# tprodanov/locityper

Hardware: AMD Instinct MI355X
Metric: reads/s through the whole genotyping path (scored + prefiltered + default solver scheme); reads_scored_per_s and genotypes_solved_per_s give the two halves (higher is better)
Workload: dtype f64

## Files before the change

### locityper_amd/csrc/lcty_api.hip

```cpp
#include <algorithm>
#include <cmath>
#include <memory>
#include <numeric>

#include "lcty_objects.hpp"

using namespace lcty;

namespace lcty {
static thread_local std::string g_last_error;
thread_local hipStream_t tl_stream = nullptr;
void set_last_error(const std::string& msg) { g_last_error = msg; }
}

hipEvent_t lcty_ctx::get_event() {
    hipEvent_t e;
    if (!event_pool.empty()) { e = event_pool.back(); event_pool.pop_back(); return e; }
    LCTY_HIP(hipEventCreate(&e));
    return e;
}

void lcty_ctx::fold_oldest(lcty::KernelTimer& t, size_t count) {
    count = std::min(count, t.pending.size());
    for (size_t i = 0; i < count; i++) {
        float ms = 0.f;
        LCTY_HIP(hipEventSynchronize(t.pending[i].second));
        LCTY_HIP(hipEventElapsedTime(&ms, t.pending[i].first, t.pending[i].second));
        t.total_ms += ms; t.launches++;
        event_pool.push_back(t.pending[i].first); event_pool.push_back(t.pending[i].second);
    }
    t.pending.erase(t.pending.begin(), t.pending.begin() + static_cast<std::ptrdiff_t>(count));
}

extern "C" {

int32_t lcty_ctx_set_knob(lcty_ctx* ctx, const char* name, int64_t value) {
    return guarded([&] {
        if (!ctx || !name) fail(LCTY_ERR_INVALID_INPUT, "null argument");
        static const char* const known[] = {"transfer_levels", "transfer_scratch_mb", "transfer_waves", "transfer_cap_new", "transfer_arena",
                                            "depth_table_start", "solve_budget_mb", "solve_chains_per_wave", "solve_extra_start", "solve_lds_weights",
                                            "anneal_lds_weights", "contig_info_slide", "gather_chunk_mb", "prefilter_gram", "prefilter_gram_cols",
                                            "prefilter_gram_levels", "comm_fail_at", "score_lean", "arena_cap_pct", "exact_threads", "host_threads",
                                            "score_lean_keep", "score_lean_two", "queue_early_head",
#ifdef LCTY_DIAG
                                            "solve_stats", "queue_trace", "map_trace", "exact_trace", "solve_greedy_form", "solve_anneal_timing", "score_timing",
                                            "solve_init_tiles", "transfer_phases",
#endif
                                            nullptr};
        bool ok = false;
        for (const char* const* k = known; *k; k++) ok |= strcmp(*k, name) == 0;
        if (!ok) fail(LCTY_ERR_INVALID_INPUT, "unknown knob '%s'", name);
        if (value < 0) ctx->knobs.erase(name); else ctx->knobs[name] = value;
    });
}

int32_t lcty_ctx_set_path(lcty_ctx* ctx, const char* name, const char* path) {
    return guarded([&] {
        if (!ctx || !name) fail(LCTY_ERR_INVALID_INPUT, "null argument");
        if (strcmp(name, "exact_dump") != 0) fail(LCTY_ERR_INVALID_INPUT, "unknown path '%s'", name);
        ctx->exact_dump_path = path ? path : "";
    });
}

const char* lcty_last_error(void) { return g_last_error.c_str(); }
const char* lcty_version(void) { return "locityper_hip 0.1.0 (gfx950)"; }

int32_t lcty_device_count(void) {
    int n = 0;
    if (hipGetDeviceCount(&n) != hipSuccess) { (void)hipGetLastError(); return 0; }
    return n;
}

int32_t lcty_ctx_create(int32_t device_id, lcty_ctx** out) {
    return guarded([&] {
        if (!out) fail(LCTY_ERR_INVALID_INPUT, "null argument");
        int n = 0;
        if (hipGetDeviceCount(&n) != hipSuccess || n == 0) {
            (void)hipGetLastError();
            fail(LCTY_ERR_RUNTIME, "no HIP device is visible: liblocityper_hip has no CPU fallback");
        }
        if (device_id < 0 || device_id >= n) fail(LCTY_ERR_INVALID_INPUT, "device %d out of range (0..%d)", device_id, n - 1);
        auto c = std::unique_ptr<lcty_ctx>(new lcty_ctx());
        c->device = device_id;
        LCTY_HIP(hipSetDevice(device_id));
        LCTY_HIP(hipGetDeviceProperties(&c->props, device_id));
        LCTY_HIP(hipStreamCreateWithFlags(&c->stream.main, hipStreamNonBlocking));
        *out = c.release();
    });
}

void lcty_ctx_destroy(lcty_ctx* ctx) {
    if (!ctx) return;
    (void)hipSetDevice(ctx->device);
    (void)hipStreamSynchronize(ctx->stream);
    for (auto& t : ctx->timers) for (auto& pr : t.pending) { (void)hipEventDestroy(pr.first); (void)hipEventDestroy(pr.second); }
    for (auto e : ctx->event_pool) (void)hipEventDestroy(e);
    if (ctx->gate.ev) (void)hipEventDestroy(ctx->gate.ev);
    if (ctx->gate.init_ev) (void)hipEventDestroy(ctx->gate.init_ev);
    if (ctx->side) { (void)hipStreamSynchronize(ctx->side); (void)hipStreamDestroy(ctx->side); }
    if (ctx->fore) { (void)hipStreamSynchronize(ctx->fore); (void)hipStreamDestroy(ctx->fore); }
    for (auto& slot : ctx->given_slots) if (slot->stream) { (void)hipStreamSynchronize(slot->stream); (void)hipStreamDestroy(slot->stream); }
    (void)hipStreamDestroy(ctx->stream.main);
    delete ctx;
}

int32_t lcty_ctx_synchronize(lcty_ctx* ctx) {
    return guarded([&] {
        if (!ctx) fail(LCTY_ERR_INVALID_INPUT, "null argument");
        ctx->activate();
        LCTY_HIP(hipStreamSynchronize(ctx->stream));
        if (ctx->side) LCTY_HIP(hipStreamSynchronize(ctx->side));
    });
}

int32_t lcty_host_alloc(lcty_ctx* ctx, uint64_t bytes, void** out) {
    return guarded([&] {
        if (!ctx || !out) fail(LCTY_ERR_INVALID_INPUT, "null argument");
        ctx->activate();
        *out = nullptr;
        LCTY_HIP(hipHostMalloc(out, std::max<uint64_t>(bytes, 1), hipHostMallocDefault));
    });
}

void lcty_host_free(void* p) {
    if (p) (void)hipHostFree(p);
}

int32_t lcty_ctx_trim(lcty_ctx* ctx) {
    return guarded([&] {
// ... 282 lines not shown
```

### locityper_amd/csrc/lcty_solve_kernels.hip

```cpp
#include <algorithm>
#include <cmath>
#include <type_traits>
#include <vector>

#include "lcty_solve_device.hpp"

namespace lcty {


__global__ __launch_bounds__(256) void build_loc_table_kernel(const uint32_t* __restrict__ good_ix, uint32_t n_good, uint64_t ngp,
                                                              uint32_t A, const uint32_t* __restrict__ pa_idx,
                                                              const uint64_t* __restrict__ pa_off, const PairAlnDev* __restrict__ pa,
                                                              const double* __restrict__ unmapped, LocCell* __restrict__ table,
                                                              uint32_t* __restrict__ table_ext, double* __restrict__ table_unm,
                                                              uint32_t* __restrict__ err) {
    __shared__ LocCell tile[32][33];
    __shared__ uint32_t tile_ext[32][33];
    const uint32_t g0 = blockIdx.x * 32, c0 = blockIdx.y * 32;
    const uint32_t tx = threadIdx.x & 31u, ty = threadIdx.x >> 5;
    if (blockIdx.y == 0 && threadIdx.x < 32) {
        const uint32_t g = g0 + threadIdx.x;
        if (g < ngp) table_unm[g] = g < n_good ? unmapped[good_ix[g]] : 0.0;
    }
    for (uint32_t i = ty; i < 32; i += 8) {
// ... 338 lines not shown
    for (uint32_t base = seg_lo; base < seg_hi; base += 64) {
        const uint32_t rp = base + lane;
        LocCell cur[P]; uint64_t at[P];
#pragma unroll
        for (uint32_t p = 0; p < P; p++) { cur[p] = nxt[p]; at[p] = row_at[p] + rp; }
        const double cur_unm = nxt_unm;
        if (rp + 64 < seg_hi) {
#pragma unroll
            for (uint32_t p = 0; p < P; p++) nxt[p] = V.table[row_at[p] + rp + 64];
            nxt_unm = V.table_unm[rp + 64];
        }
        Locs<P> L; L.nw = 0;
        uint32_t a0 = 0;
        if (rp < seg_hi) {
            locs_from_cells<P>(L, V, cur, cur_unm, at);
            if (L.nw > 255) atomicMax(V.overflow, 2u);
            if (L.nw > 1 && random_start)
                a0 = static_cast<uint32_t>(__umul64hi(counter_u64(seed ^ INIT_KEY_XOR, rp), static_cast<uint64_t>(L.nw)));
        }
        const bool nontrivial = L.nw > 1;
        const uint32_t n_extra = L.nw > 2 ? min(L.nw, 255u) - 2u : 0u;
        const unsigned long long nt_mask = __ballot(nontrivial);
        const uint32_t slot = n_recs + static_cast<uint32_t>(__popcll(nt_mask & ((1ull << lane) - 1ull)));
        n_recs += static_cast<uint32_t>(__popcll(nt_mask));
        if (L.nw > 0) {
            uint32_t eix = 0;
            if (n_extra) eix = atomicAdd(&seg_cnt[4], n_extra);
            ChainRec rec; rec.rp_cur = rp | (a0 << 24); rec.meta = min(L.nw, 255u) | (eix << 8);
            rec.lp0 = rec.lp1 = 0.0; rec.win0 = rec.win1 = 0;
            const bool room = static_cast<uint64_t>(eix) + n_extra <= V.extra_cap;
            LocIter<P> it; it.start(L);
            LocOut o;
            for (uint32_t t = 0; t < min(L.nw, 255u) && it.next(L, V, o); t++) {
                uint32_t wa, wb;
                loc_windows(V, G, o, seed, rp, t, &wa, &wb);
                const uint32_t win = wa | (wb << 16);
                if (t == 0) { rec.lp0 = o.lp; rec.win0 = win; }
                else if (t == 1) { rec.lp1 = o.lp; rec.win1 = win; }
                else if (room) { ExtraLoc e; e.lp = o.lp; e.win = win; e._pad = 0; extra[eix + t - 2] = e; }
                if (t == a0) {
                    atomicAdd(&depth[wa], 1u);
                    atomicAdd(&depth[wb], 1u);
                    aln_part += o.lp;
                }
            }
            if (nontrivial) recs[slot] = rec;
        }
    }
    if (lane == 0) seg_cnt[wave] = n_recs;
    red[tid] = aln_part;
    __syncthreads();
    const uint32_t ex_total = seg_cnt[4];
    if (tid == 0) {
        if (ex_total > V.extra_cap) { atomicMax(V.overflow, 4u); atomicMax(V.overflow + 1, ex_total); }
        if (ex_total >= (1u << 24)) atomicMax(V.overflow, 2u);
    }
    for (uint32_t s = 128; s > 0; s >>= 1) {
        if (tid < s) red[tid] += red[tid + s];
        __syncthreads();
    }
    uint32_t* gdepth = V.c_depth + static_cast<uint64_t>(chain) * V.wstride;
    for (uint32_t w = tid; w < G.total_w; w += 256) gdepth[w] = depth[w];
    if (tid == 0) {
        uint32_t* cum = V.c_seg + static_cast<uint64_t>(chain) * 4;
        uint32_t run = 0;
        for (uint32_t k = 0; k < INIT_SEGS; k++) { cum[k] = run; run += seg_cnt[k]; }
        V.c_aln[chain] = red[0]; V.c_nnt[chain] = run; V.c_totw[chain] = G.total_w;
    }
}

__device__ __forceinline__ uint64_t counter_fin(uint64_t z) {
    z = (z ^ (z >> 30)) * 0xbf58476d1ce4e5b9ull;
    z = (z ^ (z >> 27)) * 0x94d049bb133111ebull;
    return z ^ (z >> 31);
}
constexpr uint64_t GOLDEN64 = 0x9e3779b97f4a7c15ull;
typedef uint32_t u32x4_t __attribute__((ext_vector_type(4)));
__device__ __forceinline__ void store_16(uint4* p, uint4 v) {
    u32x4_t x; x.x = v.x; x.y = v.y; x.z = v.z; x.w = v.w;
    __builtin_nontemporal_store(x, reinterpret_cast<u32x4_t*>(p));
}
__host__ __device__ inline size_t init_tile_lds(uint32_t T, uint32_t R, uint32_t wstride) {
    const size_t depth = (static_cast<size_t>(T) * wstride * 4 + 15) & ~static_cast<size_t>(15);
    return depth + static_cast<size_t>(T) * 256 * 8 + 4ull * R * 64 * 16 + static_cast<size_t>(T) * 4 * 8 + static_cast<size_t>(T) * 4 * 5 + 64;
}

__device__ __forceinline__ void init_tile_deferred(const SolveView& V, const InitChainP* __restrict__ cp, uint32_t T, uint32_t* depth, double* aln_def,
                                                   uint32_t* ex_cnt, unsigned long long* queue, uint32_t head, uint32_t n, uint32_t wave, uint32_t lane, bool random_start) {
    double add = 0.0;
    uint32_t my_c = 0xFFFFFFFFu;
    if (lane < n) {
        const unsigned long long packed = __hip_atomic_load(&queue[(head + lane) & (INIT_TILE_Q - 1)], __ATOMIC_RELAXED, __HIP_MEMORY_SCOPE_WORKGROUP);
        const uint2 item = make_uint2(static_cast<uint32_t>(packed), static_cast<uint32_t>(packed >> 32));
        const uint32_t c = item.x >> 24, rp = item.x & 0xFFFFFFu, slot = item.y;
        const InitChainP P = cp[c];
        Geno<2> G;
        G.id[0] = P.id0; G.id[1] = P.id1; G.row[0] = P.row0; G.row[1] = P.row1; G.shift[0] = P.shift0; G.shift[1] = P.shift1;
        G.reg_start[0] = P.rs0; G.reg_start[1] = P.rs1; G.reg_end[0] = P.re0; G.reg_end[1] = P.re1; G.total_w = P.total_w;
        Locs<2> L;
        locs_init<2>(L, V, rp, G);
        if (L.nw > 255) atomicMax(V.overflow, 2u);
        uint32_t a0 = 0;
        if (L.nw > 1 && random_start)
            a0 = static_cast<uint32_t>(__umul64hi(counter_u64(P.seed ^ INIT_KEY_XOR, rp), static_cast<uint64_t>(L.nw)));
        const uint32_t nloc = min(L.nw, 255u), n_extra = nloc > 2 ? nloc - 2u : 0u;
        uint32_t eix = 0;
        if (n_extra) eix = atomicAdd(&ex_cnt[c], n_extra);
        const bool room = static_cast<uint64_t>(eix) + n_extra <= V.extra_cap;
        ExtraLoc* extra = V.extra + static_cast<uint64_t>(P.chain) * V.extra_cap;
        ChainRec rec; rec.rp_cur = rp | (a0 << 24); rec.meta = nloc | (eix << 8);
        rec.lp0 = rec.lp1 = 0.0; rec.win0 = rec.win1 = 0;
        LocIter<2> it; it.start(L);
        LocOut o;
        for (uint32_t t = 0; t < nloc && it.next(L, V, o); t++) {
            uint32_t wa, wb;
            loc_windows(V, G, o, P.seed, rp, t, &wa, &wb);
            const uint32_t win = wa | (wb << 16);
            if (t == 0) { rec.lp0 = o.lp; rec.win0 = win; }
            else if (t == 1) { rec.lp1 = o.lp; rec.win1 = win; }
            else if (room) { ExtraLoc e; e.lp = o.lp; e.win = win; e._pad = 0; extra[eix + t - 2] = e; }
            if (t == a0) {
                atomicAdd(&depth[static_cast<size_t>(c) * V.wstride + wa], 1u);
                atomicAdd(&depth[static_cast<size_t>(c) * V.wstride + wb], 1u);
                add = o.lp;
                my_c = c;
            }
        }
        if (L.nw > 1) V.recs[static_cast<uint64_t>(P.chain) * V.rstride + static_cast<uint64_t>(wave) * V.seg_reads + slot] = rec;
    }
    for (uint32_t c = 0; c < T; c++) {
        unsigned long long m = __ballot(my_c == c);
        if (!m) continue;
        double acc = aln_def[c * 4 + wave];
        while (m) {
            const int l = __ffsll(static_cast<long long>(m)) - 1;
            acc += __hiloint2double(__builtin_amdgcn_readlane(__double2hiint(add), l), __builtin_amdgcn_readlane(__double2loint(add), l));
            m &= m - 1;
        }
        if (lane == 0) aln_def[c * 4 + wave] = acc;
    }
}

__global__ __launch_bounds__(256) void solve_init_tile_kernel(const SolveView V, const InitGroup* __restrict__ groups, const InitChainP* __restrict__ chains,
                                                             unsigned long long* lists, const uint32_t T_max, const uint32_t R_max) {
    extern __shared__ __align__(16) uint8_t smem[];
    const uint32_t tid = threadIdx.x, lane = tid & 63u, wave = __builtin_amdgcn_readfirstlane(tid >> 6);
    const InitGroup& grp = groups[blockIdx.x];
    const uint32_t T = grp.n_chains, R = grp.n_rows;
    const InitChainP* __restrict__ cp = chains + grp.first;
    const uint32_t W = V.wstride;
    uint32_t* depth = reinterpret_cast<uint32_t*>(smem);
    size_t at = (static_cast<size_t>(T_max) * W * 4 + 15) & ~static_cast<size_t>(15);
    double* aln = reinterpret_cast<double*>(smem + at); at += static_cast<size_t>(T_max) * 256 * 8;
    uint4* stage = reinterpret_cast<uint4*>(smem + at) + static_cast<size_t>(wave) * R_max * 64; at += 4ull * R_max * 64 * 16;
    unsigned long long* queue = lists + (static_cast<size_t>(blockIdx.x) * 4 + wave) * INIT_TILE_Q;
    double* aln_def = reinterpret_cast<double*>(smem + at); at += static_cast<size_t>(T_max) * 4 * 8;
    uint32_t* ex_cnt = reinterpret_cast<uint32_t*>(smem + at); at += static_cast<size_t>(T_max) * 4;
    uint32_t* seg_cnt = reinterpret_cast<uint32_t*>(smem + at);

    for (uint32_t c = 0; c < T; c++) {
        const InitChainP P = cp[c];
        double* ww = V.c_ww + static_cast<uint64_t>(P.chain) * W;
        uint8_t* wgc = V.c_gc + static_cast<uint64_t>(P.chain) * W;
        uint32_t* wuc = V.n_wk ? V.c_uc + static_cast<uint64_t>(P.chain) * W : nullptr;
        for (uint32_t w = tid; w < P.total_w; w += 256) {
            depth[c * W + w] = 0;
            double weight = 0.0; uint32_t g = 0, uc = V.n_wk - 1;
            if (w >= 2) {
                const bool second = w >= P.shift1;
                const uint32_t allele = second ? P.id1 : P.id0, sh = second ? P.shift1 : P.shift0, rs = second ? P.rs1 : P.rs0;
                const uint32_t start = rs + (w - sh) * V.window, end = start + V.window;
                const uint32_t left = min(V.tweak, start), right = min(V.tweak, V.allele_len[allele] - end);
                const uint64_t r = counter_u64(P.seed ^ WINDOW_KEY_XOR, w);
                const int64_t off = -static_cast<int64_t>(left) + static_cast<int64_t>(__umul64hi(r, static_cast<uint64_t>(left + right + 1)));
                const uint32_t wstart = static_cast<uint32_t>(static_cast<int64_t>(start) + off);
                const uint32_t i = V.ci_off[allele] + (wstart > V.left_padding ? wstart - V.left_padding : 0u);
                weight = V.win_weight[i];
                g = V.gc[i];
                if (wuc) uc = V.uniq_cnt[i] | (static_cast<uint32_t>(V.compl_cnt[i]) << 16);
                if (weight < V.min_weight || weight < 1e-7) { weight = 0.0; g = 0; uc = V.n_wk - 1; }
            }
            ww[w] = weight; wgc[w] = static_cast<uint8_t>(g);
            if (wuc) wuc[w] = uc;
        }
        aln[c * 256 + tid] = 0.0;
        if (tid < 4) aln_def[c * 4 + tid] = 0.0;
        if (tid == 0) ex_cnt[c] = 0;
    }
    __syncthreads();

    const bool random_start = V.solver.kind == LCTY_SOLVER_ANNEAL || (V.solver.kind == LCTY_SOLVER_GREEDY && !V.solver.best_start);
    const uint32_t seg_lo = min(wave * V.seg_reads, V.n_good), seg_hi = min(seg_lo + V.seg_reads, V.n_good);
    uint64_t row_at[INIT_TILE_R];
#pragma unroll
    for (uint32_t r = 0; r < INIT_TILE_R; r++) row_at[r] = static_cast<uint64_t>(grp.row[r < R ? r : 0]) * V.ngp;
    const uint4* __restrict__ table = reinterpret_cast<const uint4*>(V.table);
    uint4 nxt[INIT_TILE_R]; double nxt_unm = 0.0;
#pragma unroll
    for (uint32_t r = 0; r < INIT_TILE_R; r++) nxt[r] = make_uint4(0, 0, 0, 0);
    if (seg_lo + lane < seg_hi) {
#pragma unroll
        for (uint32_t r = 0; r < INIT_TILE_R; r++) if (r < R) nxt[r] = table[row_at[r] + seg_lo + lane];
        nxt_unm = V.table_unm[seg_lo + lane];
    }
    uint32_t n_recs_all = 0;
    uint32_t qn = 0, qhead = 0;
    for (uint32_t base = seg_lo; base < seg_hi; base += 64) {
        const uint32_t rp = base + lane;
        const bool in = rp < seg_hi;
#pragma unroll
        for (uint32_t r = 0; r < INIT_TILE_R; r++) if (r < R) stage[r * 64 + lane] = nxt[r];
        const double unm = nxt_unm;
        if (rp + 64 < seg_hi) {
#pragma unroll
            for (uint32_t r = 0; r < INIT_TILE_R; r++) if (r < R) nxt[r] = table[row_at[r] + rp + 64];
            nxt_unm = V.table_unm[rp + 64];
        }
        const uint64_t zbase = ((static_cast<uint64_t>(rp) << 16) + 1ull) * GOLDEN64;
        const uint64_t abase = (static_cast<uint64_t>(rp) + 1ull) * GOLDEN64;
        for (uint32_t c = 0; c < T; c++) {
            const InitChainP P = cp[c];
            const uint4 qa = stage[P.ia * 64 + lane], qb = stage[P.ib * 64 + lane];
            const double aln_before = aln[c * 256 + tid];
            const double lpA = __hiloint2double(static_cast<int>(qa.y), static_cast<int>(qa.x));
            const double lpB = __hiloint2double(static_cast<int>(qb.y), static_cast<int>(qb.x));
            const uint32_t rawA = qa.z >> 24, rawB = qb.z >> 24;
            const double thresh = fmax(fmax(lpA, lpB), unm) - V.prob_diff;
            const bool kA = in && rawA != 0 && lpA >= thresh, kB = in && rawB != 0 && lpB >= thresh, kU = in && unm >= thresh;
            const bool multi = (kA && rawA > 1) || (kB && rawB > 1);
            const uint32_t nw = (kA ? 1u : 0u) + (kB ? 1u : 0u) + (kU ? 1u : 0u);
            bool nontrivial = nw > 1;
            if (__any(multi && nw == 1)) {
                if (multi && nw == 1) {
                    const uint32_t ext = V.table_ext[static_cast<uint64_t>(kA ? P.row0 : P.row1) * V.ngp + rp];
                    nontrivial = V.pa[ext].ln_prob >= thresh;
                }
            }
            const unsigned long long nt_mask = __ballot(nontrivial);
            const uint32_t before = __builtin_amdgcn_readlane(n_recs_all, c);
            const uint32_t slot = before + static_cast<uint32_t>(__popcll(nt_mask & ((1ull << lane) - 1ull)));
            {
                const uint32_t after = __builtin_amdgcn_readfirstlane(before + static_cast<uint32_t>(__popcll(nt_mask)));
                uint32_t m0_was;
                asm volatile("s_mov_b32 %1, m0\n\ts_mov_b32 m0, %3\n\tv_writelane_b32 %0, %2, m0\n\ts_mov_b32 m0, %1"
                             : "+v"(n_recs_all), "=&s"(m0_was) : "s"(after), "s"(c));
            }
            const unsigned long long mm = __ballot(multi);
            if (mm) {
                if (multi)
                    __hip_atomic_store(&queue[(qhead + qn + static_cast<uint32_t>(__popcll(mm & ((1ull << lane) - 1ull)))) & (INIT_TILE_Q - 1)],
                                       static_cast<unsigned long long>(rp | (c << 24)) | (static_cast<unsigned long long>(slot) << 32), __ATOMIC_RELAXED,
                                       __HIP_MEMORY_SCOPE_WAVEFRONT);
                qn += static_cast<uint32_t>(__popcll(mm));
            }
            const bool BgtA = lpB > lpA, UgtA = unm > lpA, UgtB = unm > lpB;
            const uint32_t posA = ((kB && BgtA) ? 1u : 0u) + ((kU && UgtA) ? 1u : 0u);
            const uint32_t posB = ((kA && !BgtA) ? 1u : 0u) + ((kU && UgtB) ? 1u : 0u);
            uint32_t tA1 = 0, tA2 = 0, tB1 = 0, tB2 = 0;
            if (V.tweak) {
                const uint64_t z0 = P.seed + zbase;
                const uint64_t rA = counter_fin(z0 + (posA == 0 ? 0ull : posA == 1 ? GOLDEN64 : 2ull * GOLDEN64));
                const uint64_t rB = counter_fin(z0 + (posB == 0 ? 0ull : posB == 1 ? GOLDEN64 : 2ull * GOLDEN64));
                tA1 = V.by_tweak.mod(static_cast<uint32_t>(rA >> 32)); tA2 = V.by_tweak.mod(static_cast<uint32_t>(rA));
                tB1 = V.by_tweak.mod(static_cast<uint32_t>(rB >> 32)); tB2 = V.by_tweak.mod(static_cast<uint32_t>(rB));
            }
            auto window_ix = [&](uint32_t mid, bool none, uint32_t tw, uint32_t rs, uint32_t re, uint32_t sh) -> uint32_t {
                const uint32_t m = mid + tw;
                uint32_t q = V.by_window.div(m - rs) + sh;
                asm volatile("" : "+v"(q));
                const uint32_t inside = (rs <= m && m < re) ? q : 1u;
                return none ? 0u : inside;
            };
            const uint32_t midA1 = qa.z & MID_NONE24, midB1 = qb.z & MID_NONE24;
            const uint32_t winA = window_ix(midA1, midA1 == MID_NONE24, tA1, P.rs0, P.re0, P.shift0) |
                                  (window_ix(qa.w, qa.w == NONE32S, tA2, P.rs0, P.re0, P.shift0) << 16);
            const uint32_t winB = window_ix(midB1, midB1 == MID_NONE24, tB1, P.rs1, P.re1, P.shift1) |
                                  (window_ix(qb.w, qb.w == NONE32S, tB2, P.rs1, P.re1, P.shift1) << 16);
            const bool a_0 = kA && posA == 0, b_0 = kB && posB == 0, a_1 = kA && posA == 1, b_1 = kB && posB == 1, a_2 = kA && posA == 2, b_2 = kB && posB == 2;
            const double lp0 = a_0 ? lpA : (b_0 ? lpB : unm), lp1 = a_1 ? lpA : (b_1 ? lpB : unm), lp2 = a_2 ? lpA : (b_2 ? lpB : unm);
            const uint32_t win0 = a_0 ? winA : (b_0 ? winB : 0u), win1 = a_1 ? winA : (b_1 ? winB : 0u), win2 = a_2 ? winA : (b_2 ? winB : 0u);
            uint32_t a0 = 0;
            double lps = lp0; uint32_t wins = win0;
            if (random_start) {
                const uint64_t r = counter_fin((P.seed ^ INIT_KEY_XOR) + abase);
                a0 = nw > 1 ? static_cast<uint32_t>(__umul64hi(r, static_cast<uint64_t>(nw))) : 0u;
                lps = a0 == 0 ? lp0 : (a0 == 1 ? lp1 : lp2); wins = a0 == 0 ? win0 : (a0 == 1 ? win1 : win2);
            }
            const bool fast = !multi && nw != 0;
            if (fast) {
                atomicAdd(&depth[c * W + (wins & 0xFFFFu)], 1u);
                atomicAdd(&depth[c * W + (wins >> 16)], 1u);
                aln[c * 256 + tid] = aln_before + lps;
            }
            uint32_t eix = 0;
            if (fast && nw == 3) {
                eix = atomicAdd(&ex_cnt[c], 1u);
                if (eix < V.extra_cap) {
                    ExtraLoc e; e.lp = lp2; e.win = win2; e._pad = 0;
                    V.extra[static_cast<uint64_t>(P.chain) * V.extra_cap + eix] = e;
                }
            }
            if (fast && nw > 1) {
                uint4* dst = reinterpret_cast<uint4*>(V.recs + static_cast<uint64_t>(P.chain) * V.rstride + static_cast<uint64_t>(wave) * V.seg_reads + slot);
                store_16(dst, make_uint4(rp | (a0 << 24), nw | (eix << 8), static_cast<uint32_t>(__double2loint(lp0)), static_cast<uint32_t>(__double2hiint(lp0))));
                store_16(dst + 1, make_uint4(static_cast<uint32_t>(__double2loint(lp1)), static_cast<uint32_t>(__double2hiint(lp1)), win0, win1));
            }
        }
        const bool last = base + 64 >= seg_hi;
        if (qn >= 64 || (last && qn)) {
            __builtin_amdgcn_fence(__ATOMIC_RELEASE, "workgroup");
            __builtin_amdgcn_wave_barrier();
            __builtin_amdgcn_fence(__ATOMIC_ACQUIRE, "workgroup");
            while (qn >= 64 || (last && qn)) {
                const uint32_t n = min(qn, 64u);
                init_tile_deferred(V, cp, T, depth, aln_def, ex_cnt, queue, qhead, n, wave, lane, random_start);
                qhead = (qhead + n) & (INIT_TILE_Q - 1); qn -= n;
            }
        }
    }
    if (lane < T) seg_cnt[lane * 4 + wave] = n_recs_all;
    __syncthreads();
    for (uint32_t c = 0; c < T; c++) {
        const InitChainP P = cp[c];
        const uint32_t ex_total = ex_cnt[c];
        if (tid == 0) {
            if (ex_total > V.extra_cap) { atomicMax(V.overflow, 4u); atomicMax(V.overflow + 1, ex_total); }
            if (ex_total >= (1u << 24)) atomicMax(V.overflow, 2u);
        }
        uint32_t* gdepth = V.c_depth + static_cast<uint64_t>(P.chain) * W;
        for (uint32_t w = tid; w < P.total_w; w += 256) gdepth[w] = depth[c * W + w];
        if (wave == 0) {
            double v = (aln[c * 256 + lane] + aln[c * 256 + 64 + lane]) + (aln[c * 256 + 128 + lane] + aln[c * 256 + 192 + lane]);
            for (int o = 32; o > 0; o >>= 1) v += __shfl_xor(v, o);
            v += (aln_def[c * 4] + aln_def[c * 4 + 1]) + (aln_def[c * 4 + 2] + aln_def[c * 4 + 3]);
            if (lane == 0) {
                uint32_t* cum = V.c_seg + static_cast<uint64_t>(P.chain) * 4;
                uint32_t run = 0;
                for (uint32_t k = 0; k < INIT_SEGS; k++) { cum[k] = run; run += seg_cnt[c * 4 + k]; }
                V.c_aln[P.chain] = v; V.c_nnt[P.chain] = run; V.c_totw[P.chain] = P.total_w;
            }
        }
    }
}

struct PairGather { int32_t c[2]; uint32_t dmax[2]; double weight[2], vnew[2], vold[2]; };
__device__ __forceinline__ double pair_term(const PairGather& g, int i, uint32_t* deepest) {
    const bool live = g.c[i] != 0 && g.weight[i] != 0.0;
    *deepest = max(*deepest, live ? g.dmax[i] : 0u);
    return live ? g.weight[i] * g.vnew[i] - g.weight[i] * g.vold[i] : 0.0;
}

__device__ __forceinline__ double lut_at(const double* lut, uint32_t index) {
    return *reinterpret_cast<const double*>(reinterpret_cast<const char*>(lut) + (index << 3));
}
constexpr uint32_t DEPTH_MASK = 0x1FFFFFFu;
struct Chain {
    const SolveView* V;
    uint32_t* wd;
    const double* ww;
    __device__ __forceinline__ double wlp(uint32_t w, uint32_t g, uint32_t d) const {
        const double weight = ww[w];
        if (weight == 0.0) return 0.0;
        if (d >= V->lut_depth) { atomicMax(V->overflow, 1u); return 0.0; }
        return weight * lut_at(V->lut, g * V->lut_depth + d);
    }
    __device__ __forceinline__ double wlp_at(uint32_t w) const { return wlp(w, wd[w] >> 25, wd[w] & DEPTH_MASK); }
    struct DepthGather { int32_t c[4]; uint32_t dmax[4]; double weight[4], vnew[4], vold[4]; };
    __device__ __forceinline__ void request(uint32_t w1, uint32_t w2, uint32_t w3, uint32_t w4, DepthGather& g) const {
        const int32_t e21 = w2 == w1, e31 = w3 == w1, e41 = w4 == w1;
        const int32_t e32 = w3 == w2, e42 = w4 == w2, e43 = w4 == w3;
        g.c[0] = -1 - e21 + e31 + e41;
        g.c[1] = e21 ? 0 : -1 + e32 + e42;
        g.c[2] = (e31 | e32) ? 0 : 1 + e43;
        g.c[3] = (e41 | e42 | e43) ? 0 : 1;
        const uint32_t w[4] = {w1, w2, w3, w4};
        uint32_t word[4];
#pragma unroll
        for (int i = 0; i < 4; i++) word[i] = wd[w[i]];
        const uint32_t last = V->lut_depth - 1;
#pragma unroll
        for (int i = 0; i < 4; i++) {
            const uint32_t d_old = word[i] & DEPTH_MASK, row = (word[i] >> 25) << V->lut_shift;
            const uint32_t d_new = static_cast<uint32_t>(static_cast<int32_t>(d_old) + g.c[i]);
            g.weight[i] = ww[w[i]];
            g.vnew[i] = lut_at(V->lut, row + min(d_new, last));
            g.vold[i] = lut_at(V->lut, row + min(d_old, last));
            g.dmax[i] = max(d_new, d_old);
        }
    }
    __device__ __forceinline__ double finish(const DepthGather& g) const {
        uint32_t deepest = 0;
        double sum = 0.0;
#pragma unroll
        for (int i = 0; i < 4; i++) {
            const bool live = g.c[i] != 0 && g.weight[i] != 0.0;
            deepest = max(deepest, live ? g.dmax[i] : 0u);
            const double term = live ? g.weight[i] * g.vnew[i] - g.weight[i] * g.vold[i] : 0.0;
            sum = i == 0 ? term : sum + term;
        }
        if (deepest > V->lut_depth - 1) atomicMax(V->overflow, 1u);
        return sum;
    }
    __device__ __forceinline__ double depth_lik_diff(uint32_t w1, uint32_t w2, uint32_t w3, uint32_t w4) const {
        DepthGather g;
        request(w1, w2, w3, w4, g);
        return finish(g);
    }
    __device__ __forceinline__ void request_pair(uint32_t wa, uint32_t wb, int32_t dir, PairGather& g) const {
        const int32_t same = wb == wa;
        g.c[0] = dir * (1 + same); g.c[1] = same ? 0 : dir;
        const uint32_t w[2] = {wa, wb};
        uint32_t word[2];
#pragma unroll
        for (int i = 0; i < 2; i++) word[i] = wd[w[i]];
        const uint32_t last = V->lut_depth - 1;
#pragma unroll
        for (int i = 0; i < 2; i++) {
            const uint32_t d_old = word[i] & DEPTH_MASK, row = (word[i] >> 25) << V->lut_shift;
            const uint32_t d_new = static_cast<uint32_t>(static_cast<int32_t>(d_old) + g.c[i]);
            g.weight[i] = ww[w[i]];
            g.vnew[i] = lut_at(V->lut, row + min(d_new, last));
            g.vold[i] = lut_at(V->lut, row + min(d_old, last));
            g.dmax[i] = max(d_new, d_old);
        }
// ... 1113 lines not shown
    }
    std::sort(gts.begin(), gts.end(), [&](uint32_t x, uint32_t y) { return key[x] != key[y] ? key[x] < key[y] : x < y; });
    auto row_of = [&](uint32_t allele) -> uint32_t { return H.row_of ? H.row_of[allele] : allele; };
    struct Unit { uint32_t gi, a0, n; };
    struct Proto { std::vector<Unit> units; uint32_t n_chains = 0, n_rows = 0; uint32_t row[8] = {0, 0, 0, 0, 0, 0, 0, 0}; };
    std::vector<Proto> protos;
    Proto cur;
    auto close = [&] { if (cur.n_chains) protos.push_back(cur); cur = Proto{}; };
    auto fresh_rows = [&](const Proto& p, uint32_t r0, uint32_t r1) -> uint32_t {
        bool h0 = false, h1 = false;
        for (uint32_t r = 0; r < p.n_rows; r++) { h0 |= p.row[r] == r0; h1 |= p.row[r] == r1; }
        return (h0 ? 0u : 1u) + ((h1 || r1 == r0) ? 0u : 1u);
    };
    auto add_rows = [&](Proto& p, uint32_t r0, uint32_t r1) {
        for (uint32_t x : {r0, r1}) {
            bool have = false;
            for (uint32_t r = 0; r < p.n_rows; r++) have |= p.row[r] == x;
            if (!have) p.row[p.n_rows++] = x;
        }
    };
    for (uint32_t gi : gts) {
        const uint32_t r0 = row_of(H.genotypes[2 * gi]), r1 = row_of(H.genotypes[2 * gi + 1]);
        for (uint32_t a0 = 0; a0 < attempts;) {
            const uint32_t want = std::min(attempts - a0, T_cap);
            if (cur.n_chains + want > T_cap || cur.n_rows + fresh_rows(cur, r0, r1) > R_cap) close();
            add_rows(cur, r0, r1);
            cur.units.push_back(Unit{gi, a0, want}); cur.n_chains += want;
            a0 += want;
        }
    }
    close();
    std::stable_sort(protos.begin(), protos.end(), [](const Proto& a, const Proto& b) { return a.n_chains > b.n_chains; });
    if (protos.size() > places) {
        uint64_t tail_chains = 0;
        for (size_t i = places; i < protos.size(); i++) tail_chains += protos[i].n_chains;
        const uint32_t piece = static_cast<uint32_t>(std::max<uint64_t>(1, std::min<uint64_t>(T_cap, tail_chains / (3 * places))));
        std::vector<Proto> tail;
        for (size_t i = places; i < protos.size(); i++) {
            Proto part;
            for (const Unit& u : protos[i].units)
                for (uint32_t done = 0; done < u.n;) {
                    const uint32_t take = std::min(u.n - done, piece - part.n_chains);
                    add_rows(part, row_of(H.genotypes[2 * u.gi]), row_of(H.genotypes[2 * u.gi + 1]));
                    part.units.push_back(Unit{u.gi, u.a0 + done, take}); part.n_chains += take;
                    done += take;
                    if (part.n_chains == piece) { tail.push_back(part); part = Proto{}; }
                }
            if (part.n_chains) tail.push_back(part);
        }
        protos.resize(places);
        protos.insert(protos.end(), tail.begin(), tail.end());
    }
    for (const Proto& p : protos) {
        InitGroup g{};
        g.first = static_cast<uint32_t>(plan.chains.size()); g.n_rows = p.n_rows;
        for (uint32_t r = 0; r < 8; r++) g.row[r] = p.row[r];
        for (const Unit& u : p.units) {
            const uint32_t id0 = H.genotypes[2 * u.gi], id1 = H.genotypes[2 * u.gi + 1];
            const uint32_t row0 = row_of(id0), row1 = row_of(id1);
            uint32_t ia = 0, ib = 0;
            for (uint32_t r = 0; r < p.n_rows; r++) { if (p.row[r] == row0) ia = r; if (p.row[r] == row1) ib = r; }
            const uint32_t nw0 = H.loc->n_windows[id0], nw1 = H.loc->n_windows[id1];
            for (uint32_t k = 0; k < u.n; k++) {
                const uint32_t chain = u.gi * attempts + u.a0 + k;
                if (chain >= nch) break;
                InitChainP P{};
                P.seed = H.seeds[chain]; P.chain = chain; P.ia = ia; P.ib = ib; P.row0 = row0; P.row1 = row1; P.id0 = id0; P.id1 = id1;
                P.shift0 = 2; P.rs0 = H.loc->reg_start[id0]; P.re0 = P.rs0 + nw0 * V.window;
                P.shift1 = 2 + nw0; P.rs1 = H.loc->reg_start[id1]; P.re1 = P.rs1 + nw1 * V.window;
                P.total_w = 2 + nw0 + nw1;
                plan.chains.push_back(P);
                g.n_chains++;
            }
        }
        if (!g.n_chains) continue;
        plan.T = std::max(plan.T, g.n_chains); plan.R = std::max(plan.R, g.n_rows);
        plan.groups.push_back(g);
    }
    plan.lds = init_tile_lds(plan.T, plan.R, V.wstride);
}

void launch_init(lcty_ctx* ctx, const SolveView& V, uint32_t nch, size_t lds_init, hipStream_t s, const InitHost* host, lcty_ctx::SolveWorkspace& ws,
                 InitPlan& plan) {
    if (V.ploidy == 2 && host && nch && ctx->diag_knob("solve_init_tiles", 1) != 0) {
        plan_init_groups(V, *host, nch, plan);
        const size_t gb = plan.groups.size() * sizeof(InitGroup), cb = plan.chains.size() * sizeof(InitChainP);
        if (ctx->diag_knob("solve_stats", 0)) {
            uint64_t rows = 0; uint32_t hist[INIT_TILE_T + 1] = {0};
            for (const InitGroup& g : plan.groups) { rows += g.n_rows; hist[g.n_chains]++; }
            fprintf(stderr, "[lcty solve] initialisation: %u chains in %zu groups (largest %u chains, %u rows; %.2f rows per chain; LDS %zu B); groups of 1..%u chains:",
                    nch, plan.groups.size(), plan.T, plan.R, static_cast<double>(rows) / nch, plan.lds, INIT_TILE_T);
            for (uint32_t t = 1; t <= INIT_TILE_T; t++) fprintf(stderr, " %u", hist[t]);
            fprintf(stderr, "\n");
        }
        const size_t lb = plan.groups.size() * 4 * INIT_TILE_Q * sizeof(unsigned long long);
        ws.init_plan.ensure_slack(gb + cb + lb);
        LCTY_HIP(hipMemcpyAsync(ws.init_plan.p, plan.groups.data(), gb, hipMemcpyHostToDevice, s));
        LCTY_HIP(hipMemcpyAsync(ws.init_plan.p + gb, plan.chains.data(), cb, hipMemcpyHostToDevice, s));
        if (plan.lds > 48 * 1024)
            LCTY_HIP(hipFuncSetAttribute(reinterpret_cast<const void*>(solve_init_tile_kernel), hipFuncAttributeMaxDynamicSharedMemorySize,
                                         static_cast<int>(plan.lds)));
        const InitGroup* d_groups = reinterpret_cast<const InitGroup*>(ws.init_plan.p);
        const InitChainP* d_chains = reinterpret_cast<const InitChainP*>(ws.init_plan.p + gb);
        ctx->timed(V.solver.kind == LCTY_SOLVER_ANNEAL ? LCTY_K_SOLVE_INIT_ANNEAL : LCTY_K_SOLVE_INIT, [&] {
            hipLaunchKernelGGL(solve_init_tile_kernel, dim3(static_cast<uint32_t>(plan.groups.size())), dim3(256), plan.lds, s, V, d_groups, d_chains,
                               reinterpret_cast<unsigned long long*>(ws.init_plan.p + gb + cb), plan.T, plan.R);
        }, s);
        LCTY_HIP(hipGetLastError());
        return;
    }
    switch (V.ploidy) {
        case 1: launch_init_p<1>(ctx, V, nch, lds_init, s); break;
        case 2: launch_init_p<2>(ctx, V, nch, lds_init, s); break;
        case 3: launch_init_p<3>(ctx, V, nch, lds_init, s); break;
        default: launch_init_p<4>(ctx, V, nch, lds_init, s); break;
    }
}
void launch_pause(hipStream_t s) { hipLaunchKernelGGL(pause_kernel, dim3(1), dim3(64), 0, s, 8u); }
void launch_store_cur(ChainRec* recs, const uint32_t* words, uint64_t n, hipStream_t s) {
    hipLaunchKernelGGL(store_cur_kernel, dim3(static_cast<uint32_t>((n + 255) / 256)), dim3(256), 0, s, recs, words, n);
    LCTY_HIP(hipGetLastError());
}
void launch_pack_rows_count(uint64_t n, const LocCell* table, uint64_t ngp, uint32_t n_good, const uint16_t* alleles, uint32_t n_rows,
                            unsigned long long* total, hipStream_t s) {
    hipLaunchKernelGGL(pack_rows_count_kernel, dim3(static_cast<uint32_t>((n + 255) / 256)), dim3(256), 0, s, table, ngp, n_good, alleles, n_rows, total);
    LCTY_HIP(hipGetLastError());
}
void launch_pack_rows(uint64_t n, const LocCell* table, const uint32_t* table_ext, const double* table_unm, uint64_t ngp, uint32_t n_good,
                      const uint16_t* alleles, uint32_t n_rows, const PairAlnDev* pa, LocEntry* cells, uint64_t out_stride, PairAlnDev* extras,
                      unsigned long long* cursor, hipStream_t s) {
    hipLaunchKernelGGL(pack_rows_kernel, dim3(static_cast<uint32_t>((n + 255) / 256)), dim3(256), 0, s, table, table_ext, table_unm, ngp, n_good, alleles,
                       n_rows, pa, cells, out_stride, extras, cursor);
    LCTY_HIP(hipGetLastError());
}
void launch_place_rows(uint64_t n, const LocEntry* cells, uint64_t in_stride, uint32_t n_good, uint32_t n_rows, uint32_t ext_base, LocCell* full,
                       uint32_t* full_ext, double* full_unm, bool write_unm, uint64_t full_stride, uint64_t first, hipStream_t s) {
    hipLaunchKernelGGL(place_rows_kernel, dim3(static_cast<uint32_t>((n + 255) / 256)), dim3(256), 0, s, cells, in_stride, n_good, n_rows, ext_base, full,
                       full_ext, full_unm, write_unm, full_stride, first);
    LCTY_HIP(hipGetLastError());
}
void launch_pad_rows(uint64_t n, LocCell* full, uint32_t* full_ext, double* full_unm, uint64_t full_stride, uint64_t from, uint32_t n_rows, hipStream_t s) {
    hipLaunchKernelGGL(pad_rows_kernel, dim3(static_cast<uint32_t>((n + 255) / 256)), dim3(256), 0, s, full, full_ext, full_unm, full_stride, from, n_rows);
    LCTY_HIP(hipGetLastError());
}
void launch_count_unexplained(uint32_t blocks, const uint8_t* status, const double* unmapped, const double* matrix, uint64_t n_pairs, uint32_t A,
                              const uint16_t* ids, uint32_t ploidy, unsigned long long* out, hipStream_t s) {
    hipLaunchKernelGGL(count_unexplained_kernel, dim3(blocks), dim3(256), 0, s, status, unmapped, matrix, n_pairs, A, ids, ploidy, out);
    LCTY_HIP(hipGetLastError());
}
void launch_read_nw(const SolveView& V, uint32_t* nw, hipStream_t s) {
    if (!V.n_good) return;
    const uint32_t blocks = (V.n_good + 255) / 256;
    switch (V.ploidy) {
        case 1: hipLaunchKernelGGL(read_nw_kernel<1>, dim3(blocks), dim3(256), 0, s, V, nw); break;
        case 2: hipLaunchKernelGGL(read_nw_kernel<2>, dim3(blocks), dim3(256), 0, s, V, nw); break;
        case 3: hipLaunchKernelGGL(read_nw_kernel<3>, dim3(blocks), dim3(256), 0, s, V, nw); break;
        default: hipLaunchKernelGGL(read_nw_kernel<4>, dim3(blocks), dim3(256), 0, s, V, nw); break;
    }
    LCTY_HIP(hipGetLastError());
}
void launch_assignment_counts(const SolveView& V, const uint32_t* nw, const uint64_t* read_off, uint16_t* counts, hipStream_t s) {
    if (!V.n_good) return;
    hipLaunchKernelGGL(assignment_counts_kernel, dim3((V.n_good + 255) / 256), dim3(256), 0, s, V, nw, read_off, counts);
    LCTY_HIP(hipGetLastError());
}

}
```

Baseline: 2.616 million.

## Keep per-chain alignment sums and record counts in registers in init tile kernel

```diff
diff --git a/locityper_amd/csrc/lcty_api.hip b/locityper_amd/csrc/lcty_api.hip
--- a/locityper_amd/csrc/lcty_api.hip
+++ b/locityper_amd/csrc/lcty_api.hip
@@ -41,10 +41,10 @@
                                             "depth_table_start", "solve_budget_mb", "solve_chains_per_wave", "solve_extra_start", "solve_lds_weights",
                                             "anneal_lds_weights", "contig_info_slide", "gather_chunk_mb", "prefilter_gram", "prefilter_gram_cols",
                                             "prefilter_gram_levels", "comm_fail_at", "score_lean", "arena_cap_pct", "exact_threads", "host_threads",
-                                            "score_lean_keep", "score_lean_two", "queue_early_head",
+                                            "score_lean_keep", "score_lean_two", "queue_early_head", "solve_init_tiles", "solve_init_per_cu",
 #ifdef LCTY_DIAG
                                             "solve_stats", "queue_trace", "map_trace", "exact_trace", "solve_greedy_form", "solve_anneal_timing", "score_timing",
-                                            "solve_init_tiles", "transfer_phases",
+                                            "transfer_phases",
 #endif
                                             nullptr};
         bool ok = false;
diff --git a/locityper_amd/csrc/lcty_solve_kernels.hip b/locityper_amd/csrc/lcty_solve_kernels.hip
--- a/locityper_amd/csrc/lcty_solve_kernels.hip
+++ b/locityper_amd/csrc/lcty_solve_kernels.hip
@@ -444,7 +444,7 @@
 }
 __host__ __device__ inline size_t init_tile_lds(uint32_t T, uint32_t R, uint32_t wstride) {
     const size_t depth = (static_cast<size_t>(T) * wstride * 4 + 15) & ~static_cast<size_t>(15);
-    return depth + static_cast<size_t>(T) * 256 * 8 + 4ull * R * 64 * 16 + static_cast<size_t>(T) * 4 * 8 + static_cast<size_t>(T) * 4 * 5 + 64;
+    return depth + 4ull * R * 64 * 16 + static_cast<size_t>(T) * 4 * 8 + static_cast<size_t>(T) * 4 * 5 + 64;
 }
 
 __device__ __forceinline__ void init_tile_deferred(const SolveView& V, const InitChainP* __restrict__ cp, uint32_t T, uint32_t* depth, double* aln_def,
@@ -513,7 +513,7 @@
     const uint32_t W = V.wstride;
     uint32_t* depth = reinterpret_cast<uint32_t*>(smem);
     size_t at = (static_cast<size_t>(T_max) * W * 4 + 15) & ~static_cast<size_t>(15);
-    double* aln = reinterpret_cast<double*>(smem + at); at += static_cast<size_t>(T_max) * 256 * 8;
+    double* red = reinterpret_cast<double*>(smem + at);
     uint4* stage = reinterpret_cast<uint4*>(smem + at) + static_cast<size_t>(wave) * R_max * 64; at += 4ull * R_max * 64 * 16;
     unsigned long long* queue = lists + (static_cast<size_t>(blockIdx.x) * 4 + wave) * INIT_TILE_Q;
     double* aln_def = reinterpret_cast<double*>(smem + at); at += static_cast<size_t>(T_max) * 4 * 8;
@@ -545,7 +545,6 @@
             ww[w] = weight; wgc[w] = static_cast<uint8_t>(g);
             if (wuc) wuc[w] = uc;
         }
-        aln[c * 256 + tid] = 0.0;
         if (tid < 4) aln_def[c * 4 + tid] = 0.0;
         if (tid == 0) ex_cnt[c] = 0;
     }
@@ -565,7 +564,10 @@
         for (uint32_t r = 0; r < INIT_TILE_R; r++) if (r < R) nxt[r] = table[row_at[r] + seg_lo + lane];
         nxt_unm = V.table_unm[seg_lo + lane];
     }
-    uint32_t n_recs_all = 0;
+    uint32_t n_recs[INIT_TILE_T];
+    double aln[INIT_TILE_T];
+#pragma unroll
+    for (uint32_t c = 0; c < INIT_TILE_T; c++) { n_recs[c] = 0; aln[c] = 0.0; }
     uint32_t qn = 0, qhead = 0;
     for (uint32_t base = seg_lo; base < seg_hi; base += 64) {
         const uint32_t rp = base + lane;
@@ -580,10 +582,11 @@
         }
         const uint64_t zbase = ((static_cast<uint64_t>(rp) << 16) + 1ull) * GOLDEN64;
         const uint64_t abase = (static_cast<uint64_t>(rp) + 1ull) * GOLDEN64;
-        for (uint32_t c = 0; c < T; c++) {
+#pragma unroll
+        for (uint32_t c = 0; c < INIT_TILE_T; c++) {
+            if (c >= T) break;
             const InitChainP P = cp[c];
             const uint4 qa = stage[P.ia * 64 + lane], qb = stage[P.ib * 64 + lane];
-            const double aln_before = aln[c * 256 + tid];
             const double lpA = __hiloint2double(static_cast<int>(qa.y), static_cast<int>(qa.x));
             const double lpB = __hiloint2double(static_cast<int>(qb.y), static_cast<int>(qb.x));
             const uint32_t rawA = qa.z >> 24, rawB = qb.z >> 24;
@@ -599,14 +602,8 @@
                 }
             }
             const unsigned long long nt_mask = __ballot(nontrivial);
-            const uint32_t before = __builtin_amdgcn_readlane(n_recs_all, c);
-            const uint32_t slot = before + static_cast<uint32_t>(__popcll(nt_mask & ((1ull << lane) - 1ull)));
-            {
-                const uint32_t after = __builtin_amdgcn_readfirstlane(before + static_cast<uint32_t>(__popcll(nt_mask)));
-                uint32_t m0_was;
-                asm volatile("s_mov_b32 %1, m0\n\ts_mov_b32 m0, %3\n\tv_writelane_b32 %0, %2, m0\n\ts_mov_b32 m0, %1"
-                             : "+v"(n_recs_all), "=&s"(m0_was) : "s"(after), "s"(c));
-            }
+            const uint32_t slot = n_recs[c] + static_cast<uint32_t>(__popcll(nt_mask & ((1ull << lane) - 1ull)));
+            n_recs[c] += static_cast<uint32_t>(__popcll(nt_mask));
             const unsigned long long mm = __ballot(multi);
             if (mm) {
                 if (multi)
@@ -652,7 +649,7 @@
             if (fast) {
                 atomicAdd(&depth[c * W + (wins & 0xFFFFu)], 1u);
                 atomicAdd(&depth[c * W + (wins >> 16)], 1u);
-                aln[c * 256 + tid] = aln_before + lps;
+                aln[c] += lps;
             }
             uint32_t eix = 0;
             if (fast && nw == 3) {
@@ -680,9 +677,14 @@
             }
         }
     }
-    if (lane < T) seg_cnt[lane * 4 + wave] = n_recs_all;
+    if (lane == 0) {
+#pragma unroll
+        for (uint32_t c = 0; c < INIT_TILE_T; c++) if (c < T) seg_cnt[c * 4 + wave] = n_recs[c];
+    }
     __syncthreads();
-    for (uint32_t c = 0; c < T; c++) {
+#pragma unroll
+    for (uint32_t c = 0; c < INIT_TILE_T; c++) {
+        if (c >= T) break;
         const InitChainP P = cp[c];
         const uint32_t ex_total = ex_cnt[c];
         if (tid == 0) {
@@ -691,8 +693,10 @@
         }
         uint32_t* gdepth = V.c_depth + static_cast<uint64_t>(P.chain) * W;
         for (uint32_t w = tid; w < P.total_w; w += 256) gdepth[w] = depth[c * W + w];
+        red[tid] = aln[c];
+        __syncthreads();
         if (wave == 0) {
-            double v = (aln[c * 256 + lane] + aln[c * 256 + 64 + lane]) + (aln[c * 256 + 128 + lane] + aln[c * 256 + 192 + lane]);
+            double v = (red[lane] + red[64 + lane]) + (red[128 + lane] + red[192 + lane]);
             for (int o = 32; o > 0; o >>= 1) v += __shfl_xor(v, o);
             v += (aln_def[c * 4] + aln_def[c * 4 + 1]) + (aln_def[c * 4 + 2] + aln_def[c * 4 + 3]);
             if (lane == 0) {
@@ -702,6 +706,7 @@
                 V.c_aln[P.chain] = v; V.c_nnt[P.chain] = run; V.c_totw[P.chain] = P.total_w;
             }
         }
+        __syncthreads();
     }
 }
 
@@ -1981,8 +1986,10 @@
 
 void launch_init(lcty_ctx* ctx, const SolveView& V, uint32_t nch, size_t lds_init, hipStream_t s, const InitHost* host, lcty_ctx::SolveWorkspace& ws,
                  InitPlan& plan) {
-    if (V.ploidy == 2 && host && nch && ctx->diag_knob("solve_init_tiles", 1) != 0) {
-        plan_init_groups(V, *host, nch, plan);
+    if (V.ploidy == 2 && host && nch && ctx->knob("solve_init_tiles", 1) != 0) {
+        InitHost h = *host;
+        if (!h.lds_budget) h.lds_budget = static_cast<uint32_t>(160 * 1024 / std::max<int64_t>(1, std::min<int64_t>(4, ctx->knob("solve_init_per_cu", 2))));
+        plan_init_groups(V, h, nch, plan);
         const size_t gb = plan.groups.size() * sizeof(InitGroup), cb = plan.chains.size() * sizeof(InitChainP);
         if (ctx->diag_knob("solve_stats", 0)) {
             uint64_t rows = 0; uint32_t hist[INIT_TILE_T + 1] = {0};
```

After: 2.621 million, median of 6. No clear change (+0.2%).
